# OpenMined/PIR

Measured on AMD Instinct MI355X. Metric: PIR queries/sec (ms/query in ms_per_step), N=4096 DB=2^20 x 288B d=2, higher is better.
Workload: dtype u64; 1 GPU; N=4096, 2 RNS data primes (36,36 bit | special 37 bit), t=24 bit, DB=2^20 x 288B, d=2, dims=[162, 162], num_pt=26215, 64 queries/step (whole job), 16 in flight per GPU (BASELINE.json configs[2]); workers=16, dist_mode=single, exchange=none, parallelism=single GPU, database_copies_in_hbm=operand layout only (u64 staging released)

## Files before the change

### pir_amd/csrc/scan_mfma.hip

```cpp
#include <hip/hip_runtime.h>

#include <stdlib.h>

#include <algorithm>

#include "arith.h"
#include "kernels.h"

namespace pirgpu {

typedef int v4i __attribute__((ext_vector_type(4)));
typedef unsigned __int128 u128;

#ifndef PIRGPU_SCAN_DIRECT
#define PIRGPU_SCAN_DIRECT 0
#endif
#ifndef PIRGPU_SCAN_PAD
#define PIRGPU_SCAN_PAD 1
#endif

__host__ __device__ __forceinline__ size_t db_tile_offset(uint32_t j, uint32_t rt, uint32_t kg, uint32_t a, uint32_t TB,
                                                          uint32_t RT, uint32_t KG, uint32_t GC) {
  const uint32_t ch = kg / GC, kg0 = ch * GC;
  const uint32_t gc = KG - kg0 < GC ? KG - kg0 : GC;
  return ((size_t)j * RT * KG + (size_t)RT * kg0 + (size_t)rt * gc + (kg - kg0)) * TB + (size_t)a * 256;
}

template <int L>
__host__ __device__ __forceinline__ constexpr int64_t top4_vmax() {
  int64_t p = 1;
  for (int a = 0; a < L - 1; ++a) p *= 256;
  return 7 * p + 127 * ((p - 1) / 255);
}
__host__ __device__ __forceinline__ constexpr uint32_t tile_bytes(uint32_t L, bool top4) {
  return top4 ? (L - 1) * 256 + 128 : L * 256;
}
typedef int v2i __attribute__((ext_vector_type(2)));
__device__ __forceinline__ uint32_t sx4(uint32_t v) {
  return v | (((v >> 3) & 0x01010101u) * 0xF0u);
}
__device__ __forceinline__ v4i expand_top4(v2i w) {
  const uint32_t w0 = (uint32_t)w[0], w1 = (uint32_t)w[1];
  return v4i{(int)sx4(w0 & 0x0F0F0F0Fu), (int)sx4((w0 >> 4) & 0x0F0F0F0Fu), (int)sx4(w1 & 0x0F0F0F0Fu),
              (int)sx4((w1 >> 4) & 0x0F0F0F0Fu)};
}
__device__ __forceinline__ v2i pack_top4(const uint8_t (&o)[16]) {
  uint32_t w[2] = {0, 0};
#pragma unroll
  for (int h = 0; h < 2; ++h)
#pragma unroll
    for (int i = 0; i < 4; ++i)
      w[h] |= (uint32_t)((o[8 * h + i] & 0xF) | ((o[8 * h + 4 + i] & 0xF) << 4)) << (8 * i);
  return v2i{(int)w[0], (int)w[1]};
}

template <int L, bool TOP4 = false>
__device__ __forceinline__ void to_digits(uint64_t x, uint64_t q, int8_t (&d)[L]) {
  int64_t v = TOP4 ? ((int64_t)x > top4_vmax<L>() ? (int64_t)x - (int64_t)q : (int64_t)x)
                   : (x > (q >> 1) ? (int64_t)x - (int64_t)q : (int64_t)x);
#pragma unroll
  for (int a = 0; a < L; ++a) {
    d[a] = (int8_t)(v & 0xFF);
    v = (v - d[a]) >> 8;
  }
}

template <int L, bool TOP4>
__global__ void __launch_bounds__(256)
db_pack_band_kernel(const DevParams* __restrict__ P, const uint64_t* __restrict__ db, uint8_t* __restrict__ dbp,
                    uint64_t npts, uint32_t cols, uint32_t kN, uint32_t rt0, uint32_t RT, uint32_t KG, uint32_t GC,
                    uint32_t slot0) {
  constexpr uint32_t TB = tile_bytes(L, TOP4);
  const uint32_t j = slot0 + blockIdx.x * 16 + (threadIdx.x & 15);
  const uint32_t r16 = threadIdx.x >> 4;
  const uint32_t rt = rt0 + blockIdx.y, kg = blockIdx.z;
  const uint32_t r = blockIdx.y * 16 + r16;
  const uint64_t q = P->mod[j >> P->logN].q;
  uint64_t x[16];
#pragma unroll
  for (int t = 0; t < 16; ++t) {
    const uint32_t c = kg * 16 + t;
    const uint64_t pt = (uint64_t)r * cols + c;
    x[t] = 0;
    if (c < cols && pt < npts) x[t] = db[pt * kN + j];
  }
  constexpr int LF = TOP4 ? L - 1 : L;
  uint32_t w[LF][4] = {};
  uint32_t w4[2] = {0, 0};
#pragma unroll
  for (int t = 0; t < 16; ++t) {
    int8_t d[L];
    to_digits<L, TOP4>(x[t], q, d);
#pragma unroll
    for (int a = 0; a < LF; ++a) w[a][t >> 2] |= (uint32_t)(uint8_t)d[a] << (8 * (t & 3));
    if constexpr (TOP4) w4[t >> 3] |= ((uint32_t)d[L - 1] & 0xFu) << (8 * (t & 3) + ((t & 4) ? 4 : 0));
  }
  uint8_t* blk = dbp + db_tile_offset(j - slot0, rt, kg, 0, TB, RT, KG, GC);
#pragma unroll
  for (int a = 0; a < LF; ++a)
    *reinterpret_cast<v4i*>(blk + (size_t)a * 256 + r16 * 16) = v4i{(int)w[a][0], (int)w[a][1], (int)w[a][2], (int)w[a][3]};
  if constexpr (TOP4) *reinterpret_cast<v2i*>(blk + (size_t)(L - 1) * 256 + r16 * 8) = v2i{(int)w4[0], (int)w4[1]};
}

template <int L, bool TOP4>
__global__ void __launch_bounds__(256)
sel_pack_kernel(const DevParams* __restrict__ P, MfmaPtrs sv, uint32_t nq, uint8_t* __restrict__ selp, uint32_t cols,
                uint32_t kN, uint32_t KG, int sel_f64, SliceMap map) {
  constexpr uint32_t TB = tile_bytes(L, TOP4);
  const uint32_t j = blockIdx.x * 16 + (threadIdx.x & 15);
  const uint32_t x = threadIdx.x >> 4;
  const uint32_t kg = blockIdx.y;
  const uint64_t q = P->mod[j >> P->logN].q;
  const uint32_t qi = x >> 1, comp = x & 1;
  if (qi >= nq) return;
  const uint64_t* src = (const uint64_t*)sv.p[qi];
  uint8_t o[L][16];
#pragma unroll
  for (int t = 0; t < 16; ++t) {
    const uint32_t c = kg * 16 + t;
    uint64_t v = 0;
    if (c < cols) v = src[((size_t)c * 2 + comp) * kN + j];
    if (sel_f64) v = f64_to_u64(__longlong_as_double((long long)v));
    int8_t d[L];
    to_digits<L, TOP4>(v, q, d);
#pragma unroll
    for (int b = 0; b < L; ++b) o[b][t] = (uint8_t)d[b];
  }
  uint32_t jl = j;
  size_t piece = 0;
  if (map.n) {
    uint32_t r = 0;
    while (r + 1 < map.n && j >= map.cut[r + 1]) ++r;
    jl = j - map.cut[r];
    piece = map.off[r];
  }
  uint8_t* blk = selp + piece + ((size_t)jl * KG + kg) * TB;
#pragma unroll
  for (int b = 0; b < L; ++b) {
    if (TOP4 && b == L - 1) {
      *reinterpret_cast<v2i*>(blk + b * 256 + x * 8) = pack_top4(o[b]);
    } else {
      v4i v;
      __builtin_memcpy(&v, o[b], 16);
      *reinterpret_cast<v4i*>(blk + b * 256 + x * 16) = v;
    }
  }
}

template <int L, bool TOP4>
__global__ void __launch_bounds__(256)
db_unpack_kernel(const DevParams* __restrict__ P, const uint8_t* __restrict__ dbp, uint64_t* __restrict__ out,
                 uint32_t r, uint32_t c, uint32_t kN, uint32_t RT, uint32_t KG, uint32_t GC) {
  constexpr uint32_t TB = tile_bytes(L, TOP4);
  const uint32_t j = blockIdx.x * 256 + threadIdx.x;
  if (j >= kN) return;
  const uint64_t q = P->mod[j >> P->logN].q;
  const uint8_t* blk = dbp + db_tile_offset(j, r >> 4, c >> 4, 0, TB, RT, KG, GC);
  const uint8_t* p = blk + (r & 15) * 16 + (c & 15);
  int64_t v = 0;
#pragma unroll
  for (int a = L - 1; a >= 0; --a) {
    if (TOP4 && a == L - 1) {
      const uint32_t cc = c & 15;
      const uint8_t byte = blk[(size_t)a * 256 + (r & 15) * 8 + (cc >> 3) * 4 + (cc & 3)];
      const int nib = (cc & 4) ? (byte >> 4) : (byte & 0xF);
      v = nib >= 8 ? nib - 16 : nib;
    } else {
      v = v * 256 + (int8_t)p[(size_t)a * 256];
    }
  }
  out[j] = v < 0 ? (uint64_t)(v + (int64_t)q) : (uint64_t)v;
}

__device__ __forceinline__ int row_byte(const uint32_t (&w)[4], int c) { return (int8_t)(w[c >> 2] >> (8 * (c & 3))); }
__device__ __forceinline__ int row_nibble(const uint32_t (&w)[2], int c) {
  const int nib = (int)(w[c >> 3] >> (8 * (c & 3) + ((c & 4) ? 4 : 0))) & 0xF;
  return nib >= 8 ? nib - 16 : nib;
}

template <int L, bool TOP4>
__global__ void __launch_bounds__(256)
db_gather_kernel(const DevParams* __restrict__ P, const uint8_t* __restrict__ dbp, const DbUnit* __restrict__ units,
                 uint64_t* __restrict__ out, uint32_t N, uint32_t RT, uint32_t KG, uint32_t GC) {
  constexpr uint32_t TB = tile_bytes(L, TOP4);
  constexpr int LF = TOP4 ? L - 1 : L;
  const uint32_t j = blockIdx.x * 256 + threadIdx.x;
  if (j >= N) return;
  const DbUnit u = units[blockIdx.y];
  const uint64_t q = P->mod[0].q;
  const uint8_t* blk = dbp + db_tile_offset(j, u.r >> 4, u.kg, 0, TB, RT, KG, GC);
  const uint32_t r16 = u.r & 15;
  uint32_t w[LF][4];
#pragma unroll
  for (int a = 0; a < LF; ++a) {
    const v4i v = *reinterpret_cast<const v4i*>(blk + (size_t)a * 256 + r16 * 16);
#pragma unroll
    for (int x = 0; x < 4; ++x) w[a][x] = (uint32_t)v[x];
  }
  uint32_t w4[2] = {0, 0};
  if constexpr (TOP4) {
    const v2i v = *reinterpret_cast<const v2i*>(blk + (size_t)(L - 1) * 256 + r16 * 8);
    w4[0] = (uint32_t)v[0];
    w4[1] = (uint32_t)v[1];
  }
  uint32_t rank = 0;
#pragma unroll
  for (int cc = 0; cc < 16; ++cc) {
    if (!((u.mask >> cc) & 1)) continue;
    int64_t v = TOP4 ? row_nibble(w4, cc) : row_byte(w[L - 1], cc);
#pragma unroll
    for (int a = L - 2; a >= 0; --a) v = v * 256 + row_byte(w[a], cc);
    out[(size_t)(u.out0 + rank) * N + j] = v < 0 ? (uint64_t)(v + (int64_t)q) : (uint64_t)v;
    ++rank;
  }
}

template <int L, bool TOP4>
__global__ void __launch_bounds__(256)
db_pack_update_kernel(const DevParams* __restrict__ P, const uint64_t* __restrict__ enc, const DbUnit* __restrict__ units,
                      uint8_t* __restrict__ dbp, uint32_t kN, uint32_t slot0, uint32_t nslots, uint32_t RT, uint32_t KG,
                      uint32_t GC) {
  constexpr uint32_t TB = tile_bytes(L, TOP4);
  constexpr int LF = TOP4 ? L - 1 : L;
  const uint32_t jl = blockIdx.x * 256 + threadIdx.x;
  if (jl >= nslots) return;
  const uint32_t j = slot0 + jl;
  const DbUnit u = units[blockIdx.y];
  const uint64_t q = P->mod[j >> P->logN].q;
  uint8_t* blk = dbp + db_tile_offset(jl, u.r >> 4, u.kg, 0, TB, RT, KG, GC);
  const uint32_t r16 = u.r & 15;
  uint32_t w[LF][4];
#pragma unroll
  for (int a = 0; a < LF; ++a) {
    const v4i v = *reinterpret_cast<const v4i*>(blk + (size_t)a * 256 + r16 * 16);
#pragma unroll
    for (int x = 0; x < 4; ++x) w[a][x] = (uint32_t)v[x];
  }
  uint32_t w4[2] = {0, 0};
  if constexpr (TOP4) {
    const v2i v = *reinterpret_cast<const v2i*>(blk + (size_t)(L - 1) * 256 + r16 * 8);
    w4[0] = (uint32_t)v[0];
    w4[1] = (uint32_t)v[1];
  }
  uint32_t rank = 0;
#pragma unroll
  for (int cc = 0; cc < 16; ++cc) {
    if (!((u.mask >> cc) & 1)) continue;
    int8_t d[L];
    to_digits<L, TOP4>(enc[(size_t)(u.out0 + rank) * kN + j], q, d);
    ++rank;
    const uint32_t sh = 8 * (cc & 3);
#pragma unroll
    for (int a = 0; a < LF; ++a) w[a][cc >> 2] = (w[a][cc >> 2] & ~(0xFFu << sh)) | ((uint32_t)(uint8_t)d[a] << sh);
    if constexpr (TOP4) {
      const uint32_t ns = sh + ((cc & 4) ? 4 : 0);
      w4[cc >> 3] = (w4[cc >> 3] & ~(0xFu << ns)) | (((uint32_t)d[L - 1] & 0xFu) << ns);
    }
  }
#pragma unroll
  for (int a = 0; a < LF; ++a)
    *reinterpret_cast<v4i*>(blk + (size_t)a * 256 + r16 * 16) = v4i{(int)w[a][0], (int)w[a][1], (int)w[a][2], (int)w[a][3]};
  if constexpr (TOP4)
    *reinterpret_cast<v2i*>(blk + (size_t)(L - 1) * 256 + r16 * 8) = v2i{(int)w4[0], (int)w4[1]};
}

__device__ __forceinline__ v4i load_tile(const uint8_t* p) {
  return __builtin_nontemporal_load(reinterpret_cast<const v4i*>(p));
}
__device__ __forceinline__ v2i load_tile8(const uint8_t* p) {
  return __builtin_nontemporal_load(reinterpret_cast<const v2i*>(p));
}

struct ChunkPlan {
  uint32_t first[kMaxScanChunks + 1];
  uint32_t nchunks;
};

constexpr int kBiasBits = 59;

#define PIRGPU_SCAN_DB_OF(g_) dbp
template <int L, int KS, int NW, bool TOP4, bool F64F = false>
__global__ void __launch_bounds__(NW * 64)
scan_mfma_kernel(const DevParams* __restrict__ P, const uint8_t* __restrict__ dbp, ScanGroups grp, uint32_t rows,
                 uint32_t RT, uint32_t KG, uint64_t chunk_stride, ChunkPlan plan, uint32_t GC, uint32_t slot0,
                 uint32_t nslots, uint64_t out_qstride, uint32_t out_rstride, uint32_t blk_major) {
#include "scan_mfma_body.inc"
}
#undef PIRGPU_SCAN_DB_OF

#define PIRGPU_SCAN_DB_OF(g_) grp.db[g_]
template <int L, int KS, int NW, bool TOP4, bool F64F = false>
__global__ void __launch_bounds__(NW * 64)
scan_mfma_runs_kernel(const DevParams* __restrict__ P, ScanGroupsDb grp, uint32_t rows, uint32_t RT, uint32_t KG,
                      uint64_t chunk_stride, ChunkPlan plan, uint32_t GC, uint32_t nslots, uint64_t out_qstride) {
  constexpr uint32_t slot0 = 0, blk_major = 0;
  const uint32_t out_rstride = nslots;
#include "scan_mfma_body.inc"
}
#undef PIRGPU_SCAN_DB_OF

__global__ void __launch_bounds__(256)
slots_assemble_kernel(const uint64_t* __restrict__ src, uint64_t* __restrict__ dst, SliceMap map, uint32_t RC, uint32_t kN,
                      uint64_t dst_qstride, uint32_t nq_total, uint32_t q0) {
  const uint32_t j = (blockIdx.x * 256 + threadIdx.x) * 2;
  const uint32_t rc = blockIdx.y, q = blockIdx.z;
  if (j >= kN) return;
  uint32_t h = 0;
  while (h + 1 < map.n && j >= map.cut[h + 1]) ++h;
  const uint32_t c0 = map.cut[h], width = map.cut[h + 1] - c0;
  typedef unsigned long long u64x2 __attribute__((ext_vector_type(2)));
  const uint64_t* s = src + (size_t)nq_total * RC * c0 + ((size_t)(q0 + q) * RC + rc) * width + (j - c0);
  *reinterpret_cast<u64x2*>(dst + (size_t)q * dst_qstride + (size_t)rc * kN + j) =
      __builtin_nontemporal_load(reinterpret_cast<const u64x2*>(s));
}


MfmaGeom mfma_geometry(const DevParams& hp, uint32_t rows, uint32_t cols, int wide_override, bool allow_top4) {
  MfmaGeom gm{};
  uint32_t bits = 0;
  for (uint32_t i = 0; i < hp.k; ++i) bits = std::max<uint32_t>(bits, 64 - (uint32_t)__builtin_clzll(hp.mod[i].q));
  if (bits <= 39) gm.L = 5;
  else if (bits <= 47) gm.L = 6;
  else if (bits <= 55) gm.L = 7;
  else return gm;
  if (rows < 1 || cols < 1) { gm.L = 0; return gm; }
  gm.RT = (rows + 15) / 16;
  gm.KG = (cols + 15) / 16;
  const uint32_t steps = (gm.KG + 3) / 4;
  const uint32_t narrow_ks = gm.L <= 6 ? 3 : 2, wide_ks = gm.L <= 6 ? 7 : 6;
  bool wide = steps > narrow_ks;
  if (wide_override >= 0) wide = wide_override != 0;
  gm.NW = wide ? 4 : 8;
  const uint32_t max_ks = wide ? wide_ks : narrow_ks;
  gm.KS = std::min(max_ks, steps);
  gm.nchunks = (steps + gm.KS - 1) / gm.KS;
  if (gm.nchunks > (uint32_t)kMaxScanChunks) { gm.L = 0; return gm; }
  gm.GC = (gm.KG + gm.nchunks - 1) / gm.nchunks;
  gm.KS = (gm.GC + 3) / 4;
  if (wide && gm.KS < 3) gm.NW = 8;
  gm.top4 = allow_top4 && gm.L <= 6 && bits <= 8 * (gm.L - 1) + 4 ? 1 : 0;
  gm.tile_bytes = tile_bytes(gm.L, gm.top4 != 0);
  const size_t kN = (size_t)hp.k * hp.N;
  gm.db_bytes = kN * gm.RT * gm.KG * gm.tile_bytes;
  gm.sel_bytes = kN * gm.KG * gm.tile_bytes;
  return gm;
}

hipError_t launch_db_pack(hipStream_t st, const DevParams* P, const MfmaGeom& gm, const uint64_t* db, uint8_t* dbp,
                          uint32_t rows, uint32_t cols, uint32_t kN, uint32_t slot0, uint32_t nslots) {
  return launch_db_pack_band(st, P, gm, db, dbp, 0, gm.RT, (uint64_t)rows * cols, cols, kN, slot0, nslots);
}

hipError_t launch_db_pack_band(hipStream_t st, const DevParams* P, const MfmaGeom& gm, const uint64_t* band, uint8_t* dbp,
                               uint32_t rt0, uint32_t n_rt, uint64_t npts, uint32_t cols, uint32_t kN, uint32_t slot0,
                               uint32_t nslots) {
  if (nslots == 0) nslots = kN - slot0;
  if (slot0 % 16 || nslots % 16 || slot0 + nslots > kN) return hipErrorInvalidValue;
  if (!n_rt || n_rt > 65535 || rt0 > gm.RT || n_rt > gm.RT - rt0 || (cols + 15) / 16 != gm.KG ||
      npts > (uint64_t)n_rt * 16 * cols)
    return hipErrorInvalidValue;
  const dim3 grid(nslots / 16, n_rt, gm.KG);
#define PIRGPU_DBPACK(L_, T_)                                                                                      \
  hipLaunchKernelGGL((db_pack_band_kernel<L_, T_>), grid, dim3(256), 0, st, P, band, dbp, npts, cols, kN, rt0, gm.RT, \
                     gm.KG, gm.GC, slot0)
  switch (gm.L) {
    case 5:
      if (gm.top4) PIRGPU_DBPACK(5, true);
      else PIRGPU_DBPACK(5, false);
      break;
    case 6:
      if (gm.top4) PIRGPU_DBPACK(6, true);
      else PIRGPU_DBPACK(6, false);
      break;
    case 7: PIRGPU_DBPACK(7, false); break;
    default: return hipErrorInvalidValue;
  }
#undef PIRGPU_DBPACK
  return hipGetLastError();
}

hipError_t launch_db_unpack(hipStream_t st, const DevParams* P, const MfmaGeom& gm, const uint8_t* dbp, uint64_t* out,
                            uint32_t row, uint32_t col, uint32_t kN) {
  const dim3 grid((kN + 255) / 256);
  switch (gm.L) {
    case 5:
      if (gm.top4) hipLaunchKernelGGL((db_unpack_kernel<5, true>), grid, dim3(256), 0, st, P, dbp, out, row, col, kN, gm.RT, gm.KG, gm.GC);
      else hipLaunchKernelGGL((db_unpack_kernel<5, false>), grid, dim3(256), 0, st, P, dbp, out, row, col, kN, gm.RT, gm.KG, gm.GC);
      break;
    case 6:
      if (gm.top4) hipLaunchKernelGGL((db_unpack_kernel<6, true>), grid, dim3(256), 0, st, P, dbp, out, row, col, kN, gm.RT, gm.KG, gm.GC);
      else hipLaunchKernelGGL((db_unpack_kernel<6, false>), grid, dim3(256), 0, st, P, dbp, out, row, col, kN, gm.RT, gm.KG, gm.GC);
      break;
    case 7: hipLaunchKernelGGL((db_unpack_kernel<7, false>), grid, dim3(256), 0, st, P, dbp, out, row, col, kN, gm.RT, gm.KG, gm.GC); break;
    default: return hipErrorInvalidValue;
  }
  return hipGetLastError();
}

hipError_t launch_db_gather(hipStream_t st, const DevParams* P, const MfmaGeom& gm, const uint8_t* dbp,
                            const DbUnit* units, uint32_t n_units, uint64_t* out, uint32_t N) {
  if (!n_units) return hipSuccess;
  if (n_units > 65535) return hipErrorInvalidValue;
  const dim3 grid((N + 255) / 256, n_units);
#define PIRGPU_DBGATHER(L_, T_) \
  hipLaunchKernelGGL((db_gather_kernel<L_, T_>), grid, dim3(256), 0, st, P, dbp, units, out, N, gm.RT, gm.KG, gm.GC)
  switch (gm.L) {
    case 5:
      if (gm.top4) PIRGPU_DBGATHER(5, true);
      else PIRGPU_DBGATHER(5, false);
      break;
    case 6:
      if (gm.top4) PIRGPU_DBGATHER(6, true);
      else PIRGPU_DBGATHER(6, false);
      break;
    case 7: PIRGPU_DBGATHER(7, false); break;
    default: return hipErrorInvalidValue;
  }
#undef PIRGPU_DBGATHER
  return hipGetLastError();
}

hipError_t launch_db_pack_update(hipStream_t st, const DevParams* P, const MfmaGeom& gm, const uint64_t* enc,
                                 const DbUnit* units, uint32_t n_units, uint8_t* dbp, uint32_t kN, uint32_t slot0,
                                 uint32_t nslots) {
  if (!n_units) return hipSuccess;
  if (nslots == 0) nslots = kN - slot0;
  if (n_units > 65535 || slot0 % 16 || nslots % 16 || slot0 + nslots > kN) return hipErrorInvalidValue;
  const dim3 grid((nslots + 255) / 256, n_units);
#define PIRGPU_DBPACKUPD(L_, T_)                                                                                    \
  hipLaunchKernelGGL((db_pack_update_kernel<L_, T_>), grid, dim3(256), 0, st, P, enc, units, dbp, kN, slot0, nslots, \
                     gm.RT, gm.KG, gm.GC)
  switch (gm.L) {
    case 5:
      if (gm.top4) PIRGPU_DBPACKUPD(5, true);
      else PIRGPU_DBPACKUPD(5, false);
      break;
    case 6:
      if (gm.top4) PIRGPU_DBPACKUPD(6, true);
      else PIRGPU_DBPACKUPD(6, false);
      break;
    case 7: PIRGPU_DBPACKUPD(7, false); break;
    default: return hipErrorInvalidValue;
  }
#undef PIRGPU_DBPACKUPD
  return hipGetLastError();
}

hipError_t launch_sel_pack(hipStream_t st, const DevParams* P, const MfmaGeom& gm, const MfmaPtrs& sv, uint32_t nq,
                           uint8_t* selp, uint32_t cols, uint32_t kN, bool sel_f64, const SliceMap* map) {
  const int f = sel_f64 ? 1 : 0;
  const dim3 grid(kN / 16, gm.KG);
  SliceMap m{};
  if (map) {
    m = *map;
    if (m.n > (uint32_t)kMaxSlices || m.cut[0] != 0 || m.cut[m.n] != kN) return hipErrorInvalidValue;
    for (uint32_t r = 0; r <= m.n; ++r)
      if (m.cut[r] % 16) return hipErrorInvalidValue;
  }
#define PIRGPU_SELPACK(L_, T_) \
  hipLaunchKernelGGL((sel_pack_kernel<L_, T_>), grid, dim3(256), 0, st, P, sv, nq, selp, cols, kN, gm.KG, f, m)
  switch (gm.L) {
    case 5:
      if (gm.top4) PIRGPU_SELPACK(5, true);
      else PIRGPU_SELPACK(5, false);
      break;
    case 6:
      if (gm.top4) PIRGPU_SELPACK(6, true);
      else PIRGPU_SELPACK(6, false);
      break;
    case 7: PIRGPU_SELPACK(7, false); break;
    default: return hipErrorInvalidValue;
  }
#undef PIRGPU_SELPACK
  return hipGetLastError();
}

hipError_t launch_slots_assemble(hipStream_t st, const uint64_t* src, uint64_t* dst, const SliceMap& map, uint32_t RC,
                                 uint32_t kN, uint32_t nq, uint64_t dst_qstride, uint32_t nq_total, uint32_t q0) {
  if (map.n == 0 || map.n > (uint32_t)kMaxSlices || map.cut[0] != 0 || map.cut[map.n] != kN || q0 + nq > nq_total)
    return hipErrorInvalidValue;
  hipLaunchKernelGGL(slots_assemble_kernel, dim3((kN / 2 + 255) / 256, RC, nq), dim3(256), 0, st, src, dst, map, RC, kN,
                     dst_qstride, nq_total, q0);
  return hipGetLastError();
}

static uint32_t scan_wgs_all() {
  static const uint32_t wgs_all = [] {
    const char* v = pirgpu_env("PIRGPU_SCAN_MFMA_WGS");
    if (v && *v) return (uint32_t)strtoul(v, nullptr, 10);
    hipDeviceProp_t prop;
    int dev = 0;
    if (hipGetDevice(&dev) != hipSuccess || hipGetDeviceProperties(&prop, dev) != hipSuccess) return 256u;
    return (uint32_t)prop.multiProcessorCount;
  }();
  return wgs_all;
}

template <int L, int KS, int NW, bool TOP4, bool F64F>
static void launch_scan_mfma_variant(hipStream_t st, const DevParams* P, const MfmaGeom& gm, const uint8_t* dbp,
                                     const ScanGroups& grp, uint32_t rows, uint64_t chunk_stride, uint32_t wgs_req,
                                     uint32_t slot0, uint32_t nslots, uint64_t out_qstride, uint32_t out_rstride,
                                     bool blk_major) {
  const uint32_t wgs = wgs_req ? std::min(wgs_req, scan_wgs_all()) : scan_wgs_all();
  ChunkPlan plan{};
  plan.nchunks = gm.nchunks;
  const uint32_t units = nslots / NW * std::max<uint32_t>(grp.n, 1);
  const uint32_t share = std::min<uint32_t>(units, std::max<uint32_t>(1, wgs / std::min<uint32_t>(gm.nchunks, wgs)));
  for (uint32_t c = 0; c <= gm.nchunks; ++c) plan.first[c] = c * share;
  hipLaunchKernelGGL((scan_mfma_kernel<L, KS, NW, TOP4, F64F>), dim3(gm.nchunks * share), dim3(NW * 64), 0, st, P, dbp, grp,
                     rows, gm.RT, gm.KG, chunk_stride, plan, gm.GC, slot0, nslots, out_qstride, out_rstride,
                     blk_major ? 1u : 0u);
}

hipError_t launch_scan_mfma_groups(hipStream_t st, const DevParams* P, const MfmaGeom& gm, const uint8_t* dbp,
                                   const ScanGroups& grp, uint32_t rows, uint64_t chunk_stride, uint32_t wgs, bool f64_fold,
                                   uint32_t slot0, uint32_t nslots, uint64_t out_qstride, uint32_t out_rstride, bool blk_major) {
  if (grp.n == 0 || grp.n > (uint32_t)kMaxScanGroups || nslots == 0 || nslots % gm.NW) return hipErrorInvalidValue;
#define PIRGPU_MFMA_ARGS st, P, gm, dbp, grp, rows, chunk_stride, wgs, slot0, nslots, out_qstride, out_rstride, blk_major
#define PIRGPU_MFMA_CASE(L_, KS_, NW_)                                                                    \
  if (gm.L == L_ && gm.KS == KS_ && gm.NW == NW_) {                                                                 \
    if constexpr (L_ <= 6) {                                                                                         \
      if (gm.top4) {                                                                                                 \
        if (f64_fold) launch_scan_mfma_variant<L_, KS_, NW_, true, true>(PIRGPU_MFMA_ARGS);                          \
        else launch_scan_mfma_variant<L_, KS_, NW_, true, false>(PIRGPU_MFMA_ARGS);                                  \
        return hipGetLastError();                                                                                    \
      }                                                                                                              \
    }                                                                                                                \
    if (gm.top4) return hipErrorInvalidValue;                                                                        \
    if (f64_fold) launch_scan_mfma_variant<L_, KS_, NW_, false, true>(PIRGPU_MFMA_ARGS);                             \
    else launch_scan_mfma_variant<L_, KS_, NW_, false, false>(PIRGPU_MFMA_ARGS);                                     \
    return hipGetLastError();                                                                                        \
  }
  PIRGPU_MFMA_CASE(5, 1, 8) PIRGPU_MFMA_CASE(5, 2, 8) PIRGPU_MFMA_CASE(5, 3, 8)
  PIRGPU_MFMA_CASE(6, 1, 8) PIRGPU_MFMA_CASE(6, 2, 8) PIRGPU_MFMA_CASE(6, 3, 8)
  PIRGPU_MFMA_CASE(7, 1, 8) PIRGPU_MFMA_CASE(7, 2, 8)
  PIRGPU_MFMA_CASE(5, 3, 4) PIRGPU_MFMA_CASE(5, 4, 4) PIRGPU_MFMA_CASE(5, 5, 4) PIRGPU_MFMA_CASE(5, 6, 4) PIRGPU_MFMA_CASE(5, 7, 4)
  PIRGPU_MFMA_CASE(6, 3, 4) PIRGPU_MFMA_CASE(6, 4, 4) PIRGPU_MFMA_CASE(6, 5, 4) PIRGPU_MFMA_CASE(6, 6, 4) PIRGPU_MFMA_CASE(6, 7, 4)
  PIRGPU_MFMA_CASE(7, 3, 4) PIRGPU_MFMA_CASE(7, 4, 4) PIRGPU_MFMA_CASE(7, 5, 4) PIRGPU_MFMA_CASE(7, 6, 4)
#undef PIRGPU_MFMA_CASE
#undef PIRGPU_MFMA_ARGS
  return hipErrorInvalidValue;
}

bool scan_mfma_runs_supported(const MfmaGeom& gm) {
  return gm.L >= 5 && gm.L <= 7 && gm.NW == 8 && gm.KS >= 1 && gm.KS <= (gm.L == 5 ? 3u : 2u);
}

template <int L, int KS, bool TOP4, bool F64F>
static void launch_scan_mfma_runs_variant(hipStream_t st, const DevParams* P, const MfmaGeom& gm, const ScanGroupsDb& grp,
                                          uint32_t rows, uint64_t chunk_stride, uint32_t wgs_req, uint32_t kN,
                                          uint64_t out_qstride) {
  constexpr int NW = 8;
  const uint32_t wgs = wgs_req ? std::min(wgs_req, scan_wgs_all()) : scan_wgs_all();
  ChunkPlan plan{};
  plan.nchunks = gm.nchunks;
  const uint32_t units = kN / NW * grp.n;
  const uint32_t share = std::min<uint32_t>(units, std::max<uint32_t>(1, wgs / std::min<uint32_t>(gm.nchunks, wgs)));
  for (uint32_t c = 0; c <= gm.nchunks; ++c) plan.first[c] = c * share;
  hipLaunchKernelGGL((scan_mfma_runs_kernel<L, KS, NW, TOP4, F64F>), dim3(gm.nchunks * share), dim3(NW * 64), 0, st, P, grp,
                     rows, gm.RT, gm.KG, chunk_stride, plan, gm.GC, kN, out_qstride);
}

hipError_t launch_scan_mfma_runs(hipStream_t st, const DevParams* P, const MfmaGeom& gm, const ScanGroupsDb& grp,
                                 uint32_t rows, uint32_t kN, uint64_t chunk_stride, uint32_t wgs, bool f64_fold,
                                 uint64_t out_qstride) {
  if (grp.n == 0 || grp.n > (uint32_t)kMaxScanGroups || kN == 0 || kN % 8 || !scan_mfma_runs_supported(gm))
    return hipErrorInvalidValue;
  for (uint32_t g = 0; g < grp.n; ++g)
    if (!grp.db[g] || !grp.sel[g] || !grp.out[g] || grp.nq[g] == 0 || grp.nq[g] > kMaxMfmaQueries) return hipErrorInvalidValue;
#define PIRGPU_RUNS_ARGS st, P, gm, grp, rows, chunk_stride, wgs, kN, out_qstride
#define PIRGPU_RUNS_CASE(L_, KS_)                                                          \
  if (gm.L == L_ && gm.KS == KS_) {                                                        \
    if constexpr (L_ <= 6) {                                                               \
      if (gm.top4) {                                                                       \
        if (f64_fold) launch_scan_mfma_runs_variant<L_, KS_, true, true>(PIRGPU_RUNS_ARGS); \
        else launch_scan_mfma_runs_variant<L_, KS_, true, false>(PIRGPU_RUNS_ARGS);        \
        return hipGetLastError();                                                          \
      }                                                                                    \
    }                                                                                      \
    if (gm.top4) return hipErrorInvalidValue;                                              \
    if (f64_fold) launch_scan_mfma_runs_variant<L_, KS_, false, true>(PIRGPU_RUNS_ARGS);   \
    else launch_scan_mfma_runs_variant<L_, KS_, false, false>(PIRGPU_RUNS_ARGS);           \
    return hipGetLastError();                                                              \
  }
  PIRGPU_RUNS_CASE(5, 1) PIRGPU_RUNS_CASE(5, 2) PIRGPU_RUNS_CASE(5, 3)
  PIRGPU_RUNS_CASE(6, 1) PIRGPU_RUNS_CASE(6, 2)
  PIRGPU_RUNS_CASE(7, 1) PIRGPU_RUNS_CASE(7, 2)
#undef PIRGPU_RUNS_CASE
#undef PIRGPU_RUNS_ARGS
  return hipErrorInvalidValue;
}

hipError_t launch_scan_mfma(hipStream_t st, const DevParams* P, const MfmaGeom& gm, const uint8_t* dbp,
                            const uint8_t* selp, uint64_t* out, uint64_t out_qstride, uint32_t nq, uint32_t rows,
                            uint32_t kN, uint64_t chunk_stride, uint32_t wgs, bool f64_fold) {
  ScanGroups grp{};
  grp.n = 1;
  grp.sel[0] = selp;
  grp.out[0] = out;
  grp.nq[0] = (uint8_t)nq;
  return launch_scan_mfma_groups(st, P, gm, dbp, grp, rows, chunk_stride, wgs, f64_fold, 0, kN, out_qstride, kN, false);
}

}
```

### pir_amd/csrc/scan_mfma_body.inc

```
  constexpr uint32_t TB = tile_bytes(L, TOP4);
  constexpr int LF = TOP4 ? L - 1 : L;
  constexpr int NS = 2 * L - 1;
  constexpr int NG = (NS + 4) / 5;
  constexpr bool kDirect = PIRGPU_SCAN_DIRECT != 0;
  __shared__ __attribute__((aligned(16))) uint64_t stage[kDirect ? 1 : 2][kDirect ? 1 : 16][kDirect ? 1 : 16][NW + PIRGPU_SCAN_PAD];
  const int w = threadIdx.x >> 6, l = threadIdx.x & 63;
  const int g = l >> 4, i16 = l & 15;
  constexpr int LOGNW = NW == 8 ? 3 : 2;
  const uint32_t nblocks = nslots >> LOGNW;
  const uint32_t nunits = nblocks * grp.n;
  uint32_t ch = 0;
  while (ch + 1 < plan.nchunks && blockIdx.x >= plan.first[ch + 1]) ++ch;
  const uint32_t wg_in_chunk = blockIdx.x - plan.first[ch], wgs_in_chunk = plan.first[ch + 1] - plan.first[ch];
  const uint32_t kg0 = ch * GC;
  const uint32_t gc = KG - kg0 < GC ? KG - kg0 : GC;
  const size_t slab = (size_t)RT * KG * TB;
  const size_t chunk_base = (size_t)RT * kg0 * TB;
  const size_t rt_stride = (size_t)gc * TB;
  const uint32_t lane16 = i16 * 16, lane8 = i16 * 8;

  v4i B[KS][L], A[KS][LF];
  v2i A4[KS];
  auto load_B = [&](uint32_t gi, uint32_t jl) {
    const uint8_t* selp = grp.sel[gi];
    const uint32_t nx = 2u * grp.nq[gi];
#pragma unroll
    for (int ks = 0; ks < KS; ++ks) {
      const uint32_t gl = ks * 4 + g, kg = kg0 + gl;
      const uint8_t* blk = selp + ((size_t)jl * KG + kg) * TB;
#pragma unroll
      for (int b = 0; b < L; ++b) {
        B[ks][b] = v4i{0, 0, 0, 0};
        if (gl < gc && (uint32_t)i16 < nx) {
          if (TOP4 && b == L - 1) B[ks][b] = expand_top4(*reinterpret_cast<const v2i*>(blk + b * 256 + lane8));
          else B[ks][b] = *reinterpret_cast<const v4i*>(blk + b * 256 + lane16);
        }
      }
    }
  };
  auto load_A = [&](int ks, const uint8_t* base, uint32_t gl) {
    const uint8_t* blk = base + (size_t)gl * TB;
#pragma unroll
    for (int a = 0; a < LF; ++a) A[ks][a] = load_tile(blk + a * 256 + lane16);
    if constexpr (TOP4) A4[ks] = load_tile8(blk + (L - 1) * 256 + lane8);
  };

#define PIRGPU_UNIT_OF(uu, gi_, blk_)                                  \
  const uint32_t gi_ = blk_major ? (uu) % grp.n : (uu) / nblocks;      \
  const uint32_t blk_ = blk_major ? (uu) / grp.n : (uu) - gi_ * nblocks;
  uint32_t u = wg_in_chunk;
  if (u >= nunits) return;
  {
    PIRGPU_UNIT_OF(u, gi, blk)
    load_B(gi, blk * NW + w);
    const uint8_t* abase = PIRGPU_SCAN_DB_OF(gi) + (size_t)(blk * NW + w) * slab + chunk_base;
#pragma unroll
    for (int ks = 0; ks < KS; ++ks) {
      const uint32_t gl = ks * 4 + g;
#pragma unroll
      for (int a = 0; a < LF; ++a) A[ks][a] = v4i{0, 0, 0, 0};
      A4[ks] = v2i{0, 0};
      if (gl < gc) load_A(ks, abase, gl);
    }
  }

  uint32_t parity = 0;
  for (; u < nunits; u += wgs_in_chunk) {
    PIRGPU_UNIT_OF(u, gi, blk)
    const uint32_t j0 = blk * NW;
    const uint32_t j = slot0 + j0 + w;
    const uint32_t mi = j >> P->logN;
    const ModConst m = P->mod[mi];
    const uint32_t nx = 2u * grp.nq[gi];
    uint64_t* const obase = grp.out[gi] + ch * chunk_stride;
    const uint64_t bias = m.q << (kBiasBits - (64 - __builtin_clzll(m.q)));
    [[maybe_unused]] const F64Mod fm{P->tab[mi].qd, P->tab[mi].qinvd};
    [[maybe_unused]] const double fw0 = P->fold_w[mi][0], fw1 = P->fold_w[mi][1], fw2 = P->fold_w[mi][2];
    const uint8_t* abase = PIRGPU_SCAN_DB_OF(gi) + (size_t)(j0 + w) * slab + chunk_base;
    const uint32_t nu = u + wgs_in_chunk;
    const bool has_next = nu < nunits;
    PIRGPU_UNIT_OF(nu, ngi, nblk)
    const uint8_t* nbase = PIRGPU_SCAN_DB_OF(has_next ? ngi : gi) + (size_t)(nblk * NW + w) * slab + chunk_base;

    for (uint32_t rt = 0; rt < RT; ++rt) {
      v4i T[NS];
#pragma unroll
      for (int s = 0; s < NS; ++s) T[s] = v4i{0, 0, 0, 0};
      const bool last = rt + 1 == RT;
      const uint8_t* next_tile = last ? nbase : abase + (size_t)(rt + 1) * rt_stride;
      const bool refill = !last || has_next;
#pragma unroll
      for (int ks = 0; ks < KS; ++ks) {
        [[maybe_unused]] v4i Atop;
        if constexpr (TOP4) Atop = expand_top4(A4[ks]);
#pragma unroll
        for (int off = 0; off < L; ++off)
#pragma unroll
          for (int a = 0; a < L; ++a) {
            const int b = (a + off) % L;
            if (TOP4 && a == L - 1)
              T[a + b] = __builtin_amdgcn_mfma_i32_16x16x64_i8(Atop, B[ks][b], T[a + b], 0, 0, 0);
            else
              T[a + b] = __builtin_amdgcn_mfma_i32_16x16x64_i8(A[ks][a < LF ? a : 0], B[ks][b], T[a + b], 0, 0, 0);
          }
        const uint32_t gl = ks * 4 + g;
        if (refill && gl < gc) load_A(ks, next_tile, gl);
      }
      if (last && has_next) load_B(ngi, nblk * NW + w);
      const int buf = parity;
      parity ^= 1;
#pragma unroll
      for (int i = 0; i < 4; ++i) {
        uint64_t r = 0;
        if constexpr (F64F) {
          constexpr int NC = (NS + 3) / 4;
          double acc = 0.0;
#pragma unroll
          for (int c = NC - 1; c >= 0; --c) {
            double C = 0.0;
#pragma unroll
            for (int s = (4 * c + 3 < NS ? 4 * c + 3 : NS - 1); s >= 4 * c; --s) C = __builtin_fma(C, 256.0, (double)T[s][i]);
            if (c == 0) acc += f64_norm(C, fm);
            else acc += f64_mulmod(C, c == 1 ? fw0 : (c == 2 ? fw1 : fw2), fm);
          }
          r = f64_to_u64(f64_canon(f64_norm(acc, fm), fm));
        } else {
#pragma unroll
          for (int gq = NG - 1; gq >= 0; --gq) {
            int64_t G = 0;
#pragma unroll
            for (int s = gq * 5; s < gq * 5 + 5 && s < NS; ++s) G += (int64_t)T[s][i] << (8 * (s - gq * 5));
            if (gq == NG - 1 && NG > 1) {
              r = (uint64_t)(G + (int64_t)bias);
            } else {
              const u128 v = ((u128)r << 40) + (uint64_t)(G + (int64_t)bias);
              r = reduce128((uint64_t)v, (uint64_t)(v >> 64), m);
            }
          }
        }
        if constexpr (kDirect) {
          const uint32_t row = rt * 16 + g * 4 + i;
          if ((uint32_t)i16 < nx && row < rows)
            obase[(size_t)(i16 >> 1) * out_qstride + ((size_t)row * 2 + (i16 & 1)) * out_rstride + j0 + w] = r;
        } else {
          stage[buf][g * 4 + i][i16][w] = r;
        }
      }
      if constexpr (kDirect) continue;
      __syncthreads();
#pragma unroll
      for (int round = 0; round < 2; ++round) {
        const int run = round * 128 + (threadIdx.x >> (LOGNW - 1));
        const int part = threadIdx.x & (NW / 2 - 1);
        const int r16 = run >> 4, x = run & 15;
        const uint32_t r = rt * 16 + r16;
        if (x < (int)nx && r < rows) {
          typedef unsigned long long u64x2 __attribute__((ext_vector_type(2)));
#if PIRGPU_SCAN_PAD == 2
          const u64x2 v = *reinterpret_cast<const u64x2*>(&stage[buf][r16][x][part * 2]);
#else
          const u64x2 v = {stage[buf][r16][x][part * 2], stage[buf][r16][x][part * 2 + 1]};
#endif
          uint64_t* dst = obase + (size_t)(x >> 1) * out_qstride + ((size_t)r * 2 + (x & 1)) * out_rstride + j0 + part * 2;
          *reinterpret_cast<u64x2*>(dst) = v;
        }
      }
    }
  }
#undef PIRGPU_UNIT_OF
```

Measured before the change: 5543 queries/s.

## Defer staged output flush by one tile to overlap stores with MFMA compute

The global write-out of each staged output tile is postponed until after the next tile's MFMA work. It is done from the other half of the double-buffered LDS stage, with one final flush after the loop, so that global stores overlap matrix compute instead of sitting right after the barrier. B-operand top4 expansion is also moved out of the load path to the start of each unit, which gives the loads time to land. The warp index is made uniform with readfirstlane, and nq is read with a word load. The cost is extra live registers for the pending-flush state, which could affect occupancy.

```diff
diff --git a/pir_amd/csrc/scan_mfma.hip b/pir_amd/csrc/scan_mfma.hip
--- a/pir_amd/csrc/scan_mfma.hip
+++ b/pir_amd/csrc/scan_mfma.hip
@@ -14,6 +14,9 @@
 
 #ifndef PIRGPU_SCAN_DIRECT
 #define PIRGPU_SCAN_DIRECT 0
+#endif
+#ifndef PIRGPU_SCAN_DEFER
+#define PIRGPU_SCAN_DEFER 1
 #endif
 #ifndef PIRGPU_SCAN_PAD
 #define PIRGPU_SCAN_PAD 1
diff --git a/pir_amd/csrc/scan_mfma_body.inc b/pir_amd/csrc/scan_mfma_body.inc
--- a/pir_amd/csrc/scan_mfma_body.inc
+++ b/pir_amd/csrc/scan_mfma_body.inc
@@ -3,8 +3,9 @@
   constexpr int NS = 2 * L - 1;
   constexpr int NG = (NS + 4) / 5;
   constexpr bool kDirect = PIRGPU_SCAN_DIRECT != 0;
+  constexpr bool kDefer = PIRGPU_SCAN_DEFER != 0 && !kDirect;
   __shared__ __attribute__((aligned(16))) uint64_t stage[kDirect ? 1 : 2][kDirect ? 1 : 16][kDirect ? 1 : 16][NW + PIRGPU_SCAN_PAD];
-  const int w = threadIdx.x >> 6, l = threadIdx.x & 63;
+  const int w = __builtin_amdgcn_readfirstlane(threadIdx.x >> 6), l = threadIdx.x & 63;
   const int g = l >> 4, i16 = l & 15;
   constexpr int LOGNW = NW == 8 ? 3 : 2;
   const uint32_t nblocks = nslots >> LOGNW;
@@ -21,9 +22,14 @@
 
   v4i B[KS][L], A[KS][LF];
   v2i A4[KS];
+  auto nq_of = [&](uint32_t gi) -> uint32_t {
+    uint32_t word;
+    __builtin_memcpy(&word, &grp.nq[gi & ~3u], 4);
+    return (word >> (8 * (gi & 3u))) & 0xFFu;
+  };
   auto load_B = [&](uint32_t gi, uint32_t jl) {
     const uint8_t* selp = grp.sel[gi];
-    const uint32_t nx = 2u * grp.nq[gi];
+    const uint32_t nx = 2u * nq_of(gi);
 #pragma unroll
     for (int ks = 0; ks < KS; ++ks) {
       const uint32_t gl = ks * 4 + g, kg = kg0 + gl;
@@ -32,10 +38,20 @@
       for (int b = 0; b < L; ++b) {
         B[ks][b] = v4i{0, 0, 0, 0};
         if (gl < gc && (uint32_t)i16 < nx) {
-          if (TOP4 && b == L - 1) B[ks][b] = expand_top4(*reinterpret_cast<const v2i*>(blk + b * 256 + lane8));
-          else B[ks][b] = *reinterpret_cast<const v4i*>(blk + b * 256 + lane16);
+          if (TOP4 && b == L - 1) {
+            const v2i t = *reinterpret_cast<const v2i*>(blk + b * 256 + lane8);
+            B[ks][b] = v4i{t[0], t[1], 0, 0};
+          } else {
+            B[ks][b] = *reinterpret_cast<const v4i*>(blk + b * 256 + lane16);
+          }
         }
       }
+    }
+  };
+  auto expand_B = [&]() {
+    if constexpr (TOP4) {
+#pragma unroll
+      for (int ks = 0; ks < KS; ++ks) B[ks][L - 1] = expand_top4(v2i{B[ks][L - 1][0], B[ks][L - 1][1]});
     }
   };
   auto load_A = [&](int ks, const uint8_t* base, uint32_t gl) {
@@ -64,6 +80,28 @@
     }
   }
 
+  auto flush = [&](int buf, uint64_t* obase, uint32_t nx, uint32_t j0, uint32_t rt) {
+#pragma unroll
+    for (int round = 0; round < 2; ++round) {
+      const int run = round * 128 + (threadIdx.x >> (LOGNW - 1));
+      const int part = threadIdx.x & (NW / 2 - 1);
+      const int r16 = run >> 4, x = run & 15;
+      const uint32_t r = rt * 16 + r16;
+      if (x < (int)nx && r < rows) {
+        typedef unsigned long long u64x2 __attribute__((ext_vector_type(2)));
+#if PIRGPU_SCAN_PAD == 2
+        const u64x2 v = *reinterpret_cast<const u64x2*>(&stage[buf][r16][x][part * 2]);
+#else
+        const u64x2 v = {stage[buf][r16][x][part * 2], stage[buf][r16][x][part * 2 + 1]};
+#endif
+        uint64_t* dst = obase + (size_t)(x >> 1) * out_qstride + ((size_t)r * 2 + (x & 1)) * out_rstride + j0 + part * 2;
+        *reinterpret_cast<u64x2*>(dst) = v;
+      }
+    }
+  };
+  uint64_t* pend_obase = nullptr;
+  uint32_t pend_nx = 0, pend_j0 = 0, pend_rt = 0;
+
   uint32_t parity = 0;
   for (; u < nunits; u += wgs_in_chunk) {
     PIRGPU_UNIT_OF(u, gi, blk)
@@ -71,7 +109,7 @@
     const uint32_t j = slot0 + j0 + w;
     const uint32_t mi = j >> P->logN;
     const ModConst m = P->mod[mi];
-    const uint32_t nx = 2u * grp.nq[gi];
+    const uint32_t nx = 2u * nq_of(gi);
     uint64_t* const obase = grp.out[gi] + ch * chunk_stride;
     const uint64_t bias = m.q << (kBiasBits - (64 - __builtin_clzll(m.q)));
     [[maybe_unused]] const F64Mod fm{P->tab[mi].qd, P->tab[mi].qinvd};
@@ -81,6 +119,7 @@
     const bool has_next = nu < nunits;
     PIRGPU_UNIT_OF(nu, ngi, nblk)
     const uint8_t* nbase = PIRGPU_SCAN_DB_OF(has_next ? ngi : gi) + (size_t)(nblk * NW + w) * slab + chunk_base;
+    expand_B();
 
     for (uint32_t rt = 0; rt < RT; ++rt) {
       v4i T[NS];
@@ -109,6 +148,7 @@
       if (last && has_next) load_B(ngi, nblk * NW + w);
       const int buf = parity;
       parity ^= 1;
+      if constexpr (kDefer) flush(buf ^ 1, pend_obase, pend_nx, pend_j0, pend_rt);
 #pragma unroll
       for (int i = 0; i < 4; ++i) {
         uint64_t r = 0;
@@ -148,23 +188,15 @@
       }
       if constexpr (kDirect) continue;
       __syncthreads();
-#pragma unroll
-      for (int round = 0; round < 2; ++round) {
-        const int run = round * 128 + (threadIdx.x >> (LOGNW - 1));
-        const int part = threadIdx.x & (NW / 2 - 1);
-        const int r16 = run >> 4, x = run & 15;
-        const uint32_t r = rt * 16 + r16;
-        if (x < (int)nx && r < rows) {
-          typedef unsigned long long u64x2 __attribute__((ext_vector_type(2)));
-#if PIRGPU_SCAN_PAD == 2
-          const u64x2 v = *reinterpret_cast<const u64x2*>(&stage[buf][r16][x][part * 2]);
-#else
-          const u64x2 v = {stage[buf][r16][x][part * 2], stage[buf][r16][x][part * 2 + 1]};
-#endif
-          uint64_t* dst = obase + (size_t)(x >> 1) * out_qstride + ((size_t)r * 2 + (x & 1)) * out_rstride + j0 + part * 2;
-          *reinterpret_cast<u64x2*>(dst) = v;
-        }
+      if constexpr (kDefer) {
+        pend_obase = obase;
+        pend_nx = nx;
+        pend_j0 = j0;
+        pend_rt = rt;
+      } else {
+        flush(buf, obase, nx, j0, rt);
       }
     }
   }
+  if constexpr (kDefer) flush((int)(parity ^ 1), pend_obase, pend_nx, pend_j0, pend_rt);
 #undef PIRGPU_UNIT_OF
```

Result: no change. 5534 queries/s (-0.2%).
